# noamzilo/sed-crnn

Hardware: AMD Instinct MI355X
Metric: mel-frames/sec training throughput (seq=256, mel=40) (higher is better)
Workload: dtype f32; 1 GPU; BASELINE config 2: mono (B=128,256,40,1) per GPU, 3xConv3x3(128)+BN+ReLU+pool(1,2)+dropout0.5, BiGRU 2x128, Linear(256,1), BCEWithLogits, Adam lr 1e-3; full fit step (fwd+loss+bwd+allreduce+Adam); global_batch=128, seq_len=256, n_mels=40, parallelism=single

## Files before the change

sed_crnn_amd/csrc/conv1.hip:

```cpp
#include "common.h"

#define C1_TT 4
#define C1_MAXBLOCKS 2048

template <int CIN>
struct C1W { f32x4 w[9 * CIN]; f32x4 b; };

template <int CIN>
__device__ __forceinline__ void c1_load_w(C1W<CIN>& W, const float* __restrict__ wp, const float* __restrict__ bias,
                                          int Cout, int cg) {
#pragma unroll
    for (int tap = 0; tap < 9; ++tap)
#pragma unroll
        for (int ci = 0; ci < CIN; ++ci)
#pragma unroll
            for (int k = 0; k < 4; ++k) W.w[tap * CIN + ci][k] = wp[((size_t)tap * Cout + cg * 4 + k) * CIN + ci];
    W.b = bias ? *(const f32x4*)(bias + cg * 4) : (f32x4){0, 0, 0, 0};
}

template <int CIN>
__device__ __forceinline__ f32x4 c1_conv(const C1W<CIN>& W, const float* __restrict__ halo, int tl, int f, int F2) {
    f32x4 acc = W.b;
#pragma unroll
    for (int kh = 0; kh < 3; ++kh)
// ... 588 lines not shown
        const int k = areal[ta] ? fi : 0, tap = k / CIN, ci = k - tap * CIN, kh = tap / 3, kw = tap - kh * 3;
        aoff[ta] = areal[ta] ? ((kw + kk) * F2 + kh) * CIN + ci : hn + (fi == NK ? 0 : 1);
    }
    f32x16 acc[NFT][CT];
#pragma unroll
    for (int ta = 0; ta < NFT; ++ta)
#pragma unroll
        for (int ct = 0; ct < CT; ++ct)
#pragma unroll
            for (int j = 0; j < 16; ++j) acc[ta][ct][j] = 0.f;
    if (tid == 0) { halo[hn] = 1.f; halo[hn + 1] = 0.f; }
    for (int tile = blockIdx.x; tile < ntiles; tile += gridDim.x) {
        const int b = tile / tblocks, t0 = (tile - b * tblocks) * C1_RM_GT;
        __syncthreads();
        for (int j = tid; j < hn; j += 256) {
            int tt = j % (C1_RM_GT + 2), ff = (j / (C1_RM_GT + 2)) % F2, ci = j / ((C1_RM_GT + 2) * F2);
            const int t = t0 + tt - 1, f = ff - 1;
            float v = 0.f;
            if (t >= 0 && t < T && f >= 0 && f < F) v = x[(((size_t)b * CIN + ci) * F + f) * T + t];
            halo[(tt * F2 + ff) * CIN + ci] = v;
        }
        __syncthreads();
        const int tp = (t0 >> 1) + wave;
        if (tp < Tp) {
            const size_t prow = ((size_t)b * Tp + tp) * F;
            const float* dp = dout + prow * C + cg + i;
            const float* pp = pooled + prow * C + cg + i;
            const unsigned char* bp = bits + prow * (C >> 2) + ((cg + i) >> 2);
            const int rowbase = (2 * wave) * F2 * CIN;
            float dv[D][CT], qv[D][CT];
            unsigned bv8[D][CT];
            auto load = [&](int slot, int f) {
                const int fc = f < F ? f : F - 1;
#pragma unroll
                for (int ct = 0; ct < CT; ++ct) {
                    dv[slot][ct] = dp[(size_t)fc * C + ct * 32];
                    qv[slot][ct] = pp[(size_t)fc * C + ct * 32];
                    bv8[slot][ct] = bp[(size_t)fc * (C >> 2) + ct * 8];
                }
            };
#pragma unroll
            for (int sl = 0; sl < D; ++sl) load(sl, sl);
            for (int f0 = 0; f0 < F; f0 += D) {
#pragma unroll
                for (int sl = 0; sl < D; ++sl) {
                    const int f = f0 + sl;
                    const int base = rowbase + (f < F ? f : F - 1) * CIN;
                    float a[NFT];
#pragma unroll
                    for (int ta = 0; ta < NFT; ++ta) a[ta] = halo[areal[ta] ? base + aoff[ta] : aoff[ta]];
#pragma unroll
                    for (int ct = 0; ct < CT; ++ct) {
                        const float bv = (f < F && qv[sl][ct] > 0.f && (int)((bv8[sl][ct] >> (i & 3)) & 1u) == kk) ? dv[sl][ct] * inv_keep : 0.f;
#pragma unroll
                        for (int ta = 0; ta < NFT; ++ta)
                            acc[ta][ct] = __builtin_amdgcn_mfma_f32_32x32x2f32(a[ta], bv, acc[ta][ct], 0, 0, 0);
                    }
                    load(sl, f + D);
                }
            }
        }
    }
    float* red = smem;
#pragma unroll
    for (int ta = 0; ta < NFT; ++ta)
#pragma unroll
        for (int ct = 0; ct < CT; ++ct) {
            __syncthreads();
#pragma unroll
            for (int j = 0; j < 16; ++j) red[(wave * 32 + (j & 3) + 8 * (j >> 2) + 4 * kk) * 32 + i] = acc[ta][ct][j];
            __syncthreads();
            for (int e = tid; e < 1024; e += 256) {
                const int row = e >> 5, col = e & 31, fi = 32 * ta + row;
                if (fi <= NK) {
                    const float sum = (red[e] + red[1024 + e]) + (red[2048 + e] + red[3072 + e]);
                    partials[((size_t)blockIdx.x * C + cg + ct * 32 + col) * NV + (fi == NK ? 0 : 1 + fi)] = sum;
                }
            }
        }
}

__device__ __forceinline__ int c1_gidx(int k, int k2, int NK) { return NK + k * NK - (k * (k - 1)) / 2 + (k2 - k); }

__global__ __launch_bounds__(256) void conv1_wgrad_assemble_k(
    const float* __restrict__ part, int rows, int Cin, int C, const double* __restrict__ gram, const float* __restrict__ wp,
    const float* __restrict__ bias, const float* __restrict__ mean, const float* __restrict__ rstd, const float* __restrict__ scale,
    const float* __restrict__ sum_g, const float* __restrict__ sum_gx, double count, float* __restrict__ dw, float* __restrict__ db,
    const float* __restrict__ gamma, const float* __restrict__ beta, float* __restrict__ dgamma) {
    const int co = blockIdx.x, NK = 9 * Cin, NV = 1 + NK;
    __shared__ double sv[37];
    __shared__ double sw[4][37];
    const int lane = threadIdx.x & 63, wv = threadIdx.x >> 6;
    {
        double a[37];
#pragma unroll
        for (int v = 0; v < 37; ++v) a[v] = 0.0;
        for (int r = threadIdx.x; r < rows; r += 256) {
            const float* pr = part + ((size_t)r * C + co) * NV;
#pragma unroll
            for (int v = 0; v < 37; ++v)
                if (v < NV) a[v] += (double)pr[v];
        }
#pragma unroll
        for (int v = 0; v < 37; ++v) {
            if (v < NV) {
                const double t = wave_sum_d(a[v]);
                if (lane == 0) sw[wv][v] = t;
            }
        }
    }
    __syncthreads();
    if (threadIdx.x < NV) sv[threadIdx.x] = (sw[0][threadIdx.x] + sw[1][threadIdx.x]) + (sw[2][threadIdx.x] + sw[3][threadIdx.x]);
    __syncthreads();
    if (wv != 0) return;
    const double b = bias ? (double)bias[co] : 0.0, mu = mean[co], rs = rstd[co], sc = scale[co];
    double wr = 0.0, ws1 = 0.0;
    for (int k2 = 0; k2 < NK; ++k2) {
        const double w2 = (double)wp[((size_t)(k2 / Cin) * C + co) * Cin + (k2 % Cin)];
        ws1 += w2 * gram[k2];
        wr += w2 * sv[1 + k2];
    }
    const double sgx_sum = rs * (b * sv[0] + wr - mu * sv[0]);
    const bool own = sum_gx == nullptr;
    const double sg = (double)sum_g[co] / count, sgx = (own ? sgx_sum : (double)sum_gx[co]) / count;
    if (lane < NK) {
        const int k = lane;
        double wg = 0.0;
        for (int k2 = 0; k2 < NK; ++k2) {
            const double w2 = (double)wp[((size_t)(k2 / Cin) * C + co) * Cin + (k2 % Cin)];
            wg += w2 * gram[k <= k2 ? c1_gidx(k, k2, NK) : c1_gidx(k2, k, NK)];
        }
        const double s1 = gram[k];
        const double val = sc * (sv[1 + k] - sg * s1 - sgx * rs * (b * s1 + wg - mu * s1));
        const int tap = k / Cin, ci = k - tap * Cin;
        dw[((size_t)co * Cin + ci) * 9 + tap] = (float)val;
    }
    if (lane == 63) {
        const double sum_y = count * b + ws1;
        db[co] = (float)(sc * (sv[0] - count * sg - sgx * rs * (sum_y - count * mu)));
        if (dgamma && (own || (gamma && beta && gamma[co] == 0.f && beta[co] > 0.f))) dgamma[co] = (float)sgx_sum;
    }
}

static size_t c1_lds(int Cin, int F, int C, int mode) {
    size_t halo = (size_t)(C1_TT + 2) * (F + 2) * Cin * sizeof(float);
    size_t nv = mode == 3 ? 5 : 2;
    size_t red = (size_t)256 * 4 * nv * sizeof(float);
    return halo > red ? halo : red;
}

static int c1_shape_ok(int Cin, int F, int T, int C, int pool_f, int pool_t, int max_cin);
extern "C" int sed_conv1_fused_supported(int Cin, int F, int T, int C, int pool_f, int pool_t) {
    return c1_shape_ok(Cin, F, T, C, pool_f, pool_t, 2);
}
static int c1_shape_ok(int Cin, int F, int T, int C, int pool_f, int pool_t, int max_cin) {
    if (Cin < 1 || Cin > max_cin || C < 4 || F < 1 || T < 1 || C % 4 != 0 || C / 4 > 256 || (256 % (C / 4)) != 0) return 0;
    if (pool_t < 1 || pool_f < 1 || C1_TT % pool_t != 0 || T % C1_TT != 0 || F % pool_f != 0 || T % pool_t != 0) return 0;
    if (c1_lds(Cin, F, C, 3) > 150 * 1024) return 0;
    return 1;
}

extern "C" int sed_conv1_fused_rows(int B, int T) {
    long n = (long)B * ((T + C1_TT - 1) / C1_TT);
    return (int)(n < C1_MAXBLOCKS ? n : C1_MAXBLOCKS);
}

template <int MODE>
static int c1_launch(const float* x, const float* wp, const float* bias, const float* scale, const float* shift,
                     const float* mean, const float* rstd, const float* sum_g, const float* sum_gx, const float* dout,
                     float* out, float* partials, int B, int Cin, int F, int T, int C, int pf, int pt, float drop_p,
                     uint64_t seed, const uint64_t* seed_dev, hipStream_t s) {
    size_t lds = c1_lds(Cin, F, C, MODE);
    int grid = sed_conv1_fused_rows(B, T);
    const bool p12 = (pf == 1 && pt == 2);
#define C1_LAUNCH(CIN_, P12_)                                                                                          \
    do {                                                                                                               \
        if (lds > 48 * 1024)                                                                                           \
            (void)hipFuncSetAttribute((const void*)conv1_fused_k<CIN_, MODE, P12_>, hipFuncAttributeMaxDynamicSharedMemorySize, (int)lds); \
        conv1_fused_k<CIN_, MODE, P12_><<<grid, 256, lds, s>>>(x, wp, bias, scale, shift, mean, rstd, sum_g, sum_gx, dout, out, \
                                                              partials, B, F, T, C, pf, pt, drop_p, seed, seed_dev);  \
    } while (0)
    if (Cin == 1) { if (p12) C1_LAUNCH(1, true); else C1_LAUNCH(1, false); }
    else if (Cin == 2) { if (p12) C1_LAUNCH(2, true); else C1_LAUNCH(2, false); }
    else if ((MODE == 1 || MODE == 4) && p12) {
        if (Cin == 3) C1_LAUNCH(3, true);
        else C1_LAUNCH(4, true);
    } else {
        sed_set_error("conv1: %d input channels are supported by the forward pass with the (1,2) pool only", Cin);
        return SED_EUNSUPPORTED;
    }
#undef C1_LAUNCH
    return 0;
}
// ... 201 lines not shown
```

sed_crnn_amd/csrc/net.hip:

```cpp
#include <string.h>
#include "common.h"

namespace {

struct ConvL { int Cin, C, T, F, Tp, Fp, pf, pt, rows, bn_rows, nchw, fused; float drop;
               int red_rows;
               int rg_rows;
               int rgrad;
               int wino, wino_d;
               int ev;
               int bf; };

struct GruL { int in, H; };

struct Layout {
    int n_conv, n_gru, n_dense, M, Tp, Fp, feat;
    int proj_bf;
    ConvL cv[SED_MAX_CONV];
    GruL gr[SED_MAX_GRU];
    int dK[SED_MAX_DENSE], dN[SED_MAX_DENSE];
    size_t wp_f[SED_MAX_CONV], wp_d[SED_MAX_CONV], conv_out[SED_MAX_CONV], stat[SED_MAX_CONV];
    size_t mean[SED_MAX_CONV], rstd[SED_MAX_CONV], scale[SED_MAX_CONV], shift[SED_MAX_CONV];
    size_t pooled[SED_MAX_CONV], bn_sums[SED_MAX_CONV], c1_stat_ws, c1_bits, c1_mom;
    size_t bias_f[SED_MAX_CONV];
// ... 441 lines not shown
    for (int l = 0; l < L.n_conv; ++l) conv_bf16[l] = L.cv[l].bf;
    *proj_bf16 = L.proj_bf;
    return 0;
}

extern "C" int sed_net_routing(const sed_net_cfg* c, const sed_net_params* p, const float* x, const void* workspace, int block,
                               unsigned char* route, void* stream) {
    SED_REQUIRE(p && x && workspace && route, "net_routing: null pointer");
    Layout L;
    SED_TRY(build_layout(c, 1, &L));
    SED_REQUIRE(block >= 0 && block < L.n_conv, "net_routing: block %d out of range", block);
    const float* ws = (const float*)workspace;
    const ConvL& q = L.cv[block];
    if (q.fused) {
        SED_REQUIRE(p->conv_b[block], "net_routing: missing parameters of conv block %d", block);
        return sed_conv1_route(x, ws + L.wp_f[block], p->conv_b[block], ws + L.scale[block], ws + L.shift[block], route,
                               c->B, q.Cin, q.F, q.T, q.C, q.pf, q.pt, stream);
    }
    return sed_bn_relu_pool_route(ws + L.conv_out[block], ws + L.scale[block], ws + L.shift[block], route,
                                  c->B, q.T, q.F, q.C, q.pf, q.pt, stream);
}

static int bn_backward(const Layout& L, const sed_net_cfg* c, const sed_net_params* p, const sed_net_params* g,
                       const float* x, float* ws, uint64_t seed, const uint64_t* seed_dev, int l, int part, float count_scale, void* st) {
    const ConvL& q = L.cv[l];
    const int B = c->B, last = (l == L.n_conv - 1);
    const uint64_t sd = layer_seed(seed, l);
    SED_REQUIRE(g->conv_w[l] && g->conv_b[l] && g->bn_g[l] && g->bn_b[l], "net_backward: missing gradient buffers of conv block %d", l);
    float* sum_g = ws + L.sum_g;
    float* sum_gx = sum_g + q.C;
    if ((part & 1) && q.red_rows > 0 && !q.fused) {
        SED_TRY(sed_bn_bwd_finalize_small_gamma(ws + L.bn_part, q.red_rows, q.C, sum_g, sum_gx, g->bn_g[l], g->bn_b[l], ws + L.gradA,
                                                ws + L.pooled[l], ws + L.conv_out[l], p->bn_g[l], p->bn_b[l], ws + L.mean[l], ws + L.rstd[l],
                                                ws + L.scale[l], ws + L.shift[l], B, q.T, q.F, q.pf, q.pt, q.drop, st));
    } else if ((part & 1) && q.red_rows > 0) {
        SED_TRY(sed_bn_bwd_finalize(ws + L.bn_part, q.red_rows, q.C, sum_g, sum_gx, g->bn_g[l], g->bn_b[l], st));
    } else if (part & 1) {
        if (q.fused)
            SED_TRY(sed_conv1_bwd_reduce(x, ws + L.wp_f[l], p->conv_b[l], ws + L.gradA, ws + L.scale[l], ws + L.shift[l],
                                         ws + L.mean[l], ws + L.rstd[l], ws + L.bn_part, B, q.Cin, q.F, q.T, q.C, q.pf, q.pt,
                                         q.drop, sd, seed_dev, st));
        else if (sed_bn_bwd_reduce_pooled_supported(q.F, q.C, q.pf, q.pt, last))
            SED_TRY(sed_bn_bwd_reduce_pooled(ws + L.pooled[l], ws + L.gradA, p->bn_g[l], p->bn_b[l], ws + L.conv_out[l],
                                             ws + L.mean[l], ws + L.rstd[l], ws + L.scale[l], ws + L.shift[l], ws + L.bn_part, B, q.T, q.F, q.C, q.pf, q.pt, last, q.drop, st));
        else
            SED_TRY(sed_bn_relu_pool_drop_bwd_reduce(ws + L.conv_out[l], ws + L.gradA, ws + L.scale[l], ws + L.shift[l],
                                                     ws + L.mean[l], ws + L.rstd[l], ws + L.bn_part, B, q.T, q.F, q.C, q.pf,
                                                     q.pt, last, q.drop, sd, seed_dev, st));
        SED_TRY(sed_bn_bwd_finalize(ws + L.bn_part, q.bn_rows, q.C, sum_g, sum_gx, g->bn_g[l], g->bn_b[l], st));
    }
    if (part & 2) {
        if (count_scale != 1.f) SED_TRY(sed_scale(sum_g, 2 * q.C, 1.f / count_scale, st));
        if (q.fused && q.rgrad && q.rg_rows > 0) {
            SED_TRY(sed_conv1_bwd_wgrad_assemble(ws + L.c1_ws, q.rg_rows, (const double*)(ws + L.c1_mom), ws + L.wp_f[l], p->conv_b[l],
                                                 ws + L.mean[l], ws + L.rstd[l], ws + L.scale[l], sum_g, count_scale == 1.f ? nullptr : sum_gx, g->conv_w[l], g->conv_b[l],
                                                 B, q.Cin, q.F, q.T, q.C, p->bn_g[l], p->bn_b[l], g->bn_g[l], st));
        } else if (q.fused && q.rgrad) {
            SED_TRY(sed_conv1_bwd_wgrad(x, ws + L.gradA, ws + L.pooled[l], (const unsigned char*)(ws + L.c1_bits), (const double*)(ws + L.c1_mom),
                                        ws + L.wp_f[l], p->conv_b[l], ws + L.mean[l], ws + L.rstd[l], ws + L.scale[l], sum_g,
                                        (count_scale == 1.f && q.red_rows > 0) ? nullptr : sum_gx,
                                        g->conv_w[l], g->conv_b[l], ws + L.c1_ws, B, q.Cin, q.F, q.T, q.C, q.drop,
                                        q.red_rows > 0 ? p->bn_g[l] : nullptr, q.red_rows > 0 ? p->bn_b[l] : nullptr,
                                        q.red_rows > 0 ? g->bn_g[l] : nullptr, st));
        } else if (q.fused) {
            SED_TRY(sed_conv1_bwd_apply_wgrad(x, ws + L.wp_f[l], p->conv_b[l], ws + L.gradA, ws + L.scale[l], ws + L.shift[l],
                                              ws + L.mean[l], ws + L.rstd[l], sum_g, sum_gx, g->conv_w[l], g->conv_b[l],
                                              ws + L.c1_ws, B, q.Cin, q.F, q.T, q.C, q.pf, q.pt, q.drop, sd, seed_dev,
                                              q.red_rows > 0 ? p->bn_g[l] : nullptr, q.red_rows > 0 ? p->bn_b[l] : nullptr,
                                              q.red_rows > 0 ? g->bn_g[l] : nullptr, st));
        } else {
            SED_TRY(sed_bn_relu_pool_drop_bwd_apply(ws + L.conv_out[l], ws + L.gradA, ws + L.scale[l], ws + L.shift[l],
                                                    ws + L.mean[l], ws + L.rstd[l], sum_g, sum_gx, ws + L.dconv[l],
                                                    ws + L.dbias_part, B, q.T, q.F, q.C, q.pf, q.pt, last, q.drop, sd, seed_dev, st));
            SED_TRY(sed_reduce_rows(ws + L.dbias_part, q.bn_rows, q.C, q.C, g->conv_b[l], st));
        }
    }
    return 0;
}

static int dgrad(const Layout& L, const sed_net_cfg* c, const sed_net_params* p, const float* x, float* ws, int l, void* st) {
    const ConvL& q = L.cv[l];
    const ConvL& u = L.cv[l - 1];
    if (u.rg_rows > 0 && q.wino_d)
        return sed_conv3x3_wino_dgrad_bnred_rg(ws + L.dconv[l], ws + L.wp_d[l], ws + L.gradA, ws + L.bn_part, ws + L.pooled[l - 1],
                                               p->bn_g[l - 1], p->bn_b[l - 1], ws + L.mean[l - 1], ws + L.rstd[l - 1], u.drop,
                                               x, u.Cin, (const unsigned char*)(ws + L.c1_bits), ws + L.c1_ws, c->B, q.C, q.F, q.T, q.Cin, st);
    if (u.rg_rows > 0)
        return sed_conv3x3_dgrad_bnred_rg(ws + L.dconv[l], ws + L.wp_d[l], ws + L.gradA, ws + L.bn_part, ws + L.pooled[l - 1],
                                          p->bn_g[l - 1], p->bn_b[l - 1], ws + L.mean[l - 1], ws + L.rstd[l - 1], u.drop,
                                          x, u.Cin, (const unsigned char*)(ws + L.c1_bits), ws + L.c1_ws, c->B, q.C, q.F, q.T, q.Cin, st);
    if (q.wino_d)
        return sed_conv3x3_wino_dgrad_bnred(ws + L.dconv[l], ws + L.wp_d[l], ws + L.gradA, ws + L.bn_part, ws + L.pooled[l - 1],
                                            p->bn_g[l - 1], p->bn_b[l - 1], u.fused ? nullptr : ws + L.conv_out[l - 1],
                                            ws + L.mean[l - 1], ws + L.rstd[l - 1], u.drop, u.pf, u.pt, u.F, u.T, c->B, q.C, q.F, q.T, q.Cin, st);
    if (u.red_rows > 0)
        return sed_conv3x3_dgrad_bnred(ws + L.dconv[l], ws + L.wp_d[l], ws + L.gradA, ws + L.bn_part, ws + L.pooled[l - 1],
                                       p->bn_g[l - 1], p->bn_b[l - 1],
                                       u.fused ? nullptr : ws + L.conv_out[l - 1],
                                       ws + L.mean[l - 1], ws + L.rstd[l - 1],
                                       u.drop, u.pf, u.pt, u.F, u.T, c->B, q.C, q.F, q.T, q.Cin, st);
    return sed_conv3x3_fwd_ex(ws + L.dconv[l], 0, ws + L.wp_d[l], nullptr, ws + L.gradA, nullptr, c->B, q.C, q.F, q.T, q.Cin, c->conv_mode, st);
}

extern "C" int sed_net_backward(const sed_net_cfg* c, const sed_net_params* p, const sed_net_params* g,
                                const float* x, const float* dlogits, void* workspace, uint64_t seed,
                                const uint64_t* seed_dev, int stage_begin, int stage_end, void* stream, void* aux_stream) {
    SED_REQUIRE(p && g && x && dlogits && workspace, "net_backward: null pointer");
    constexpr int kMaxDev = 16;
    static thread_local hipEvent_t ev_all[kMaxDev][2][SED_MAX_CONV] = {};
    static thread_local hipEvent_t ev_gru_all[kMaxDev][SED_MAX_GRU + 5] = {};
    hipStream_t s_main = as_stream(stream), s_aux = as_stream(aux_stream);
    hipEvent_t* ev_dg = nullptr;
    hipEvent_t* ev_bn = nullptr;
    hipEvent_t* ev_gru = nullptr;
    if (s_aux && s_aux != s_main) {
        int dev = 0;
        if (hipGetDevice(&dev) != hipSuccess || dev < 0 || dev >= kMaxDev) {
            sed_set_error("net_backward: device index %d outside [0,%d)", dev, kMaxDev);
            return SED_EINVAL;
        }
        ev_dg = ev_all[dev][0];
        ev_bn = ev_all[dev][1];
        ev_gru = ev_gru_all[dev];
        for (int i = 0; i < SED_MAX_GRU + 5; ++i)
            if (!ev_gru[i] && hipEventCreateWithFlags(&ev_gru[i], hipEventDisableTiming) != hipSuccess) {
                sed_set_error("net_backward: hipEventCreate failed");
                return SED_EINVAL;
            }
        for (int l = 0; l < SED_MAX_CONV; ++l)
            if (!ev_dg[l]) {
                if (hipEventCreateWithFlags(&ev_dg[l], hipEventDisableTiming) != hipSuccess ||
                    hipEventCreateWithFlags(&ev_bn[l], hipEventDisableTiming) != hipSuccess) {
                    sed_set_error("net_backward: hipEventCreate failed");
                    return SED_EINVAL;
                }
            }
    } else {
        s_aux = nullptr;
    }
    Layout L;
    SED_TRY(build_layout(c, 1, &L));
    SED_REQUIRE(stage_begin >= 0 && stage_end <= L.n_conv + 1 && stage_begin < stage_end,
                "net_backward: bad stage range [%d,%d)", stage_begin, stage_end);
    float* ws = (float*)workspace;
    const int B = c->B, M = L.M;

    const int wg_clean = ((L.wgrad_zrow > 0 && s_aux) ? SED_WGRAD_ZERO_ROW_CLEAN : 0) | ((c->flags & SED_NET_DIRECT_CONV) ? SED_WGRAD_DIRECT : 0);
    if (s_aux && stage_begin == 0 && L.n_conv > 1) {
        hipError_t e = hipEventRecord(ev_gru[SED_MAX_GRU + 4], s_main);
        if (e == hipSuccess) e = hipStreamWaitEvent(s_aux, ev_gru[SED_MAX_GRU + 4], 0);
        if (e == hipSuccess) e = hipMemsetAsync(ws + L.wg_arrive, 0, (64 + L.wgrad_zrow) * sizeof(float), s_aux);
        if (e == hipSuccess && L.wgrad_zrow > 0) e = hipMemsetAsync(ws + L.wgrad_ws_aux, 0, L.wgrad_zrow * sizeof(float), s_aux);
        if (e == hipSuccess) e = hipEventRecord(ev_gru[SED_MAX_GRU + 3], s_aux);
        if (e != hipSuccess) {
            sed_set_error("net_backward: clearing the weight-gradient zero rows failed: %s", hipGetErrorString(e));
            return (int)e;
        }
    }

    if (stage_begin == 0) {
        const float* gru_last = ws + L.gout[L.n_gru - 1];
        for (int j = L.n_dense - 1; j >= 0; --j) {
            const int last = (j == L.n_dense - 1);
            const float* xin = (j == 0) ? gru_last : ws + L.act[j - 1];
            float* dy = last ? const_cast<float*>(dlogits) : ws + L.dact[j];
            float* dx = (j == 0) ? ws + L.dgout[L.n_gru - 1] : ws + L.dact[j - 1];
            SED_REQUIRE(g->dense_w[j] && g->dense_b[j], "net_backward: missing gradient buffers of dense layer %d", j);
// ... 194 lines not shown
```

sed_crnn_amd/csrc/wino.hip:

```cpp
#include "common.h"
#include "conv_shared.h"
#include <type_traits>

#define WN_CIN 128
#define WN_NHMAX 14

typedef __attribute__((address_space(1))) const void* sed_gptr_t;
typedef __attribute__((address_space(3))) void* sed_lptr_t;

struct WinoGeo {
    int Fw;
    int ncg, Tw, ntile, nblk, TR, F2, H2, HR, nb8, ncoh, NH;
    float invFw, invF2;
    size_t lds;
    unsigned long long* dbg;
};

__global__ void conv_pack_wino_k(const float* __restrict__ w, float* __restrict__ uf, float* __restrict__ ud, int Cout, int Cin,
                                 const float* __restrict__ bias, const float* __restrict__ gamma, const float* __restrict__ beta,
                                 const float* __restrict__ rm, const float* __restrict__ rv, float eps, float* __restrict__ bias_out) {
    const int i = blockIdx.x * blockDim.x + threadIdx.x;
    if (gamma && i < Cout) {
        const float sc = gamma[i] / sqrtf(rv[i] + eps);
        bias_out[i] = (bias ? bias[i] : 0.f) * sc + (beta[i] - rm[i] * sc);
// ... 75 lines not shown
    constexpr int CIN = WN_CIN, NCHUNK = CIN / 32, NSTEP = 4 * NCHUNK;
    constexpr int HBUF = NH * 1024;
    constexpr bool RG = RGC > 0;
    static_assert(!RG || BNR, "the tap sums belong to the BatchNorm-backward epilogue");
    static_assert(!EV || !BNR, "the pooling epilogue belongs to the inference forward");
    extern __shared__ __attribute__((aligned(16))) float smem[];
    const int tid = threadIdx.x, lane = tid & 63, wave = __builtin_amdgcn_readfirstlane(tid >> 6);
    const int r = lane & 31, h = lane >> 5;
    unsigned long long tk0 = 0, tk1 = 0, tk2 = 0;
    if (geo.dbg) tk0 = __builtin_amdgcn_s_memrealtime();

    int blka, coh, b;
    {
        const int bx = blockIdx.x, by = blockIdx.y, nba = geo.nblk * geo.ncg;
        if ((gridDim.y & 7) == 0) {
            const int id = by * (int)gridDim.x + bx, xcd = id & 7, j = id >> 3;
            coh = j % geo.ncoh;
            const int jj = j / geo.ncoh;
            b = xcd + 8 * (jj / nba);
            blka = jj % nba;
        } else {
            coh = bx % geo.ncoh; blka = bx / geo.ncoh; b = by;
        }
    }
    const int blk = blka / geo.ncg, cgp = blka - blk * geo.ncg;
    const int fg0 = 2 * cgp * geo.Fw;
    const int Fw = geo.Fw, F2 = geo.F2, H2 = geo.H2, ntile = geo.ntile;
    const int q0 = blk * 64, ty0 = q0 / Fw;
    const int co0 = coh * 64;

    const int ra = wave == 0 ? 0 : (wave == 2 ? 2 : 1);
    const int rb = wave == 0 ? 2 : (wave == 1 ? 2 : (wave == 2 ? 1 : 3));
    const float sg = wave == 1 ? 1.f : -1.f;

    const float* hp[NH];
    {
        const int Q = lane >> 3, pp = lane & 7;
        const float* zrow = uq + (size_t)16 * CIN * Cout;
#pragma unroll
        for (int u = 0; u < NH; ++u) {
            const int P = (u * 4 + wave) * 8 + pp;
            const int tt = sed_fdiv(P, geo.invF2), cx = P - tt * F2;
            const int ff = cx < H2 ? 2 * cx : 2 * (cx - H2) + 1;
            const int t = 2 * ty0 - 1 + tt, f = fg0 + ff - 1;
            const bool in = P < geo.HR && t >= 0 && t < T && f >= 0 && f < F;
            hp[u] = in ? x + ((((size_t)b * T + t) * F + f) * CIN + Q * 4) : zrow + Q * 4;
        }
    }
    auto issue = [&](int cc, float* buf) {
#pragma unroll
        for (int u = 0; u < NH; ++u)
            __builtin_amdgcn_global_load_lds((sed_gptr_t)(hp[u] + cc * 32), (sed_lptr_t)(buf + (u * 4 + wave) * 256), 16, 0, 0);
    };
    issue(0, smem);
    __builtin_amdgcn_sched_barrier(0);

    int aoff[2][2][4];
#pragma unroll
    for (int mt = 0; mt < 2; ++mt) {
        int q = q0 + mt * 32 + r;
        q = q < ntile ? q : ntile - 1;
        const int ty = sed_fdiv(q, geo.invFw), tf = q - ty * Fw;
#pragma unroll
        for (int s = 0; s < 2; ++s)
#pragma unroll
            for (int c = 0; c < 4; ++c) {
                const int P = (2 * (ty - ty0) + (s ? rb : ra)) * F2 + tf + (c & 1) * H2 + (c >> 1);
                aoff[mt][s][c] = (P >> 3) * 256 + h * 32 + (P & 7) * 4;
            }
    }


    unsigned* rowtab = (unsigned*)(smem + (2 * HBUF > 32768 + 512 ? 2 * HBUF : 32768 + 512));
    unsigned* xofftab = rowtab + 64;
    float* xs = (float*)(xofftab + 64);
    const int XT = 4 * geo.TR + 2;
    if (tid < 64) {
        const int q = q0 + tid;
        const int ty = sed_fdiv(q < ntile ? q : 0, geo.invFw), tf = q - ty * Fw;
        rowtab[tid] = q < ntile ? (unsigned)(((EV ? ty : 2 * ty) * F + fg0 + 2 * tf) * Cout) * 4u : 0xFFFFFFFFu;
        if (RG) xofftab[tid] = (unsigned)((fg0 + 2 * tf) * XT + 4 * (ty - ty0));
    }
    if (RG) {
        for (int i = tid; i < (F + 2) * XT; i += 256) {
            const int ff = i / XT, tt = i - ff * XT;
            const int f = ff - 1, t = 4 * ty0 - 1 + tt;
            const bool in = f >= 0 && f < F && t >= 0 && t < br.Ty;
#pragma unroll
            for (int ci = 0; ci < RGC; ++ci)
                xs[ci * (F + 2) * XT + i] = in ? br.x1[(((size_t)b * RGC + ci) * F + f) * br.Ty + t] : 0.f;
        }
    }

    f32x16 acc[4][2][2];
#pragma unroll
    for (int nu = 0; nu < 4; ++nu)
#pragma unroll
        for (int mt = 0; mt < 2; ++mt)
#pragma unroll
            for (int nt = 0; nt < 2; ++nt)
#pragma unroll
                for (int j = 0; j < 16; ++j) acc[nu][mt][nt][j] = 0.f;

    const f32x4* wl = (const f32x4*)uq + (size_t)(coh * 16 + wave * 4) * (NCHUNK * 4 * 2 * 64);
    f32x4 bq[4][2];
    const unsigned lane16 = (unsigned)lane * 16u;
    auto load_b = [&](int nu, int st) {
#pragma unroll
        for (int nt = 0; nt < 2; ++nt)
            bq[nu][nt] = *(const f32x4*)((const char*)(wl + ((nu * NSTEP + st) * 2 + nt) * 64) + lane16);
    };
    static_assert(NH <= 16, "the patch DMA of a slice rides in every fourth slot of its first step");
    f32x2 vp[2][2][4][2];
    f32x4 raw[2][2][4];
    f32x2 up[2][4][2];
    const f32x2 sg2 = {sg, sg};
    auto slot_read = [&](const float* buf, int g, int i) {
        const int mt = i >> 3, s2 = (i >> 2) & 1, c = i & 3;
        raw[mt][s2][c] = *(const f32x4*)(buf + aoff[mt][s2][c] + g * 64);
    };
    auto slot_xform = [&](int k, f32x2 (&v)[2][4][2]) {
        const int mt = k >> 4, q = k & 15, hf = q & 1;
        if (q < 8) {
            const int c = q >> 1;
            const f32x2 da = hf ? __builtin_shufflevector(raw[mt][0][c], raw[mt][0][c], 2, 3) : __builtin_shufflevector(raw[mt][0][c], raw[mt][0][c], 0, 1);
            const f32x2 db = hf ? __builtin_shufflevector(raw[mt][1][c], raw[mt][1][c], 2, 3) : __builtin_shufflevector(raw[mt][1][c], raw[mt][1][c], 0, 1);
            up[mt][c][hf] = wn_pk_fma(sg2, db, da);
        } else {
            const int nu = (q - 8) >> 1;
            if (nu == 0) v[mt][0][hf] = wn_pk_sub(up[mt][0][hf], up[mt][2][hf]);
            else if (nu == 1) v[mt][1][hf] = wn_pk_add(up[mt][1][hf], up[mt][2][hf]);
            else if (nu == 2) v[mt][2][hf] = wn_pk_sub(up[mt][2][hf], up[mt][1][hf]);
            else v[mt][3][hf] = wn_pk_sub(up[mt][1][hf], up[mt][3][hf]);
        }
    };
    auto issue_one = [&](int cc, float* buf, int u) {
        __builtin_amdgcn_global_load_lds((sed_gptr_t)(hp[u] + cc * 32), (sed_lptr_t)(buf + (u * 4 + wave) * 256), 16, 0, 0);
    };

#pragma unroll
    for (int nu = 0; nu < 4; ++nu) load_b(nu, 0);
    __syncthreads();
#pragma unroll
    for (int i = 0; i < 16; ++i) slot_read(smem, 0, i);
#pragma unroll
    for (int k = 0; k < 32; ++k) slot_xform(k, vp[0]);
    if (geo.dbg) tk1 = __builtin_amdgcn_s_memrealtime();
#pragma unroll
    for (int st = 0; st < NSTEP; ++st) {
        const int cc = st >> 2, g = st & 3, par = st & 1;
        const bool more = cc + 1 < NCHUNK, nxt = st + 1 < NSTEP;
        const float* nbuf = smem + (((st + 1) >> 2) & 1) * HBUF;
        __builtin_amdgcn_sched_barrier(0);
#pragma unroll
        for (int i = 0; i < 64; ++i) {
            const int nu = i >> 4, j = (i >> 2) & 3, mt = (i >> 1) & 1, nt = i & 1;
            acc[nu][mt][nt] = __builtin_amdgcn_mfma_f32_32x32x2f32(vp[par][mt][nu][j >> 1][j & 1], bq[nu][nt][j], acc[nu][mt][nt], 0, 0, 0);
            if (nxt && !(ABL & 4)) {
                if (i < 16) slot_read(nbuf, (st + 1) & 3, i);
                else if (i < 48 && !(ABL & 1)) slot_xform(i - 16, vp[par ^ 1]);
            }
            if (nxt && (i & 15) == 15 && !(ABL & 2)) load_b(nu, st + 1);
            if (g == 0 && more && !(ABL & 8) && (i & 3) == 1 && (i >> 2) < NH) issue_one(cc + 1, smem + ((cc + 1) & 1) * HBUF, i >> 2);
            __builtin_amdgcn_sched_barrier(0);
        }
        if (nxt && (ABL & 5)) {
#pragma unroll
            for (int a = 0; a < 2; ++a)
#pragma unroll
                for (int c = 0; c < 4; ++c) { vp[par ^ 1][a][c][0] = vp[par][a][c][0]; vp[par ^ 1][a][c][1] = vp[par][a][c][1]; }
        }
        if (g == 2 && more) __syncthreads();
    }
    __syncthreads();
    if (geo.dbg) tk2 = __builtin_amdgcn_s_memrealtime();

#pragma unroll
    for (int mt = 0; mt < 2; ++mt)
#pragma unroll
        for (int nt = 0; nt < 2; ++nt) {
            const f32x16 z0 = acc[0][mt][nt] + acc[1][mt][nt] + acc[2][mt][nt];
            const f32x16 z1 = acc[1][mt][nt] - acc[2][mt][nt] - acc[3][mt][nt];
            float* zb0 = smem + ((((wave * 2 + 0) * 2 + mt) * 2 + nt) << 10);
            float* zb1 = smem + ((((wave * 2 + 1) * 2 + mt) * 2 + nt) << 10);
#pragma unroll
            for (int j = 0; j < 16; ++j) {
                const int row = (j & 3) + 8 * (j >> 2) + 4 * h;
                zb0[row * 32 + r] = z0[j];
                zb1[row * 32 + r] = z1[j];
            }
        }
    __builtin_amdgcn_sched_barrier(0);
    const int mt = wave >> 1, nt = wave & 1;
    const int rq = lane >> 3, c4 = (lane & 7) * 4;
    const int cb = co0 + nt * 32 + c4;
    f32x4 bv = {0, 0, 0, 0};
    if (bias) bv = *(const f32x4*)(bias + cb);
    char* const yb = (char*)(y + (size_t)b * (EV ? T >> 1 : T) * F * Cout + cb);
    const char* const qb = BNR ? (const char*)(br.pooled + (size_t)b * T * F * Cout + cb) : nullptr;
    f32x4 q_kr = {0, 0, 0, 0}, q_nb = {0, 0, 0, 0}, a1 = {0, 0, 0, 0}, a2 = {0, 0, 0, 0};
    if (BNR) {
        const f32x4 q_beta = *(const f32x4*)(br.beta + cb);
        const f32x4 gm = *(const f32x4*)(br.gamma + cb);
#pragma unroll
        for (int e = 0; e < 4; ++e) {
            const bool zero = gm[e] == 0.f || (br.ybelow != nullptr && fabsf(gm[e]) * 64.f < fabsf(q_beta[e]));
            const float rg = zero ? 0.f : 1.0f / gm[e];
            q_kr[e] = br.keep * rg;
            q_nb[e] = -q_beta[e] * rg;
        }
    }
    const unsigned rstride = (unsigned)(F * Cout) * 4u, cstride = (unsigned)Cout * 4u;
    f32x4 R[RG ? 9 * RGC : 1];
#pragma unroll
    for (int k = 0; k < (RG ? 9 * RGC : 1); ++k) R[k] = (f32x4){0, 0, 0, 0};
    const unsigned char* const bitq = RG ? br.bits + (size_t)b * T * F * (Cout >> 2) + (cb >> 2) : nullptr;
    unsigned rov[4], xov[4];
#pragma unroll
    for (int k = 0; k < 4; ++k) {
        rov[k] = rowtab[mt * 32 + rq + 8 * k];
        xov[k] = RG ? xofftab[mt * 32 + rq + 8 * k] : 0u;
    }
    constexpr int PF = RGC == 2 ? 2 : 4;
    f32x4 pqv[PF][BNR ? 4 : 1];
    unsigned btv[PF][RG ? 4 : 1];
    auto prefetch = [&](int k, f32x4* pqd, unsigned* btd) {
        if (!BNR) return;
#pragma unroll
        for (int jj = 0; jj < 2; ++jj)
#pragma unroll
            for (int i = 0; i < 2; ++i) {
                const unsigned off = rov[k] + i * rstride + jj * cstride;
                pqd[jj * 2 + i] = (f32x4){0, 0, 0, 0};
                if (RG) btd[jj * 2 + i] = 0u;
                if (rov[k] != 0xFFFFFFFFu) {
                    pqd[jj * 2 + i] = *(const f32x4*)(qb + off);
                    if (RG) btd[jj * 2 + i] = bitq[off >> 4];
                }
            }
    };
    if (PF == 4) {
#pragma unroll
        for (int k = 0; k < 4; ++k) prefetch(k, pqv[k], btv[k]);
    } else prefetch(0, pqv[0], btv[0]);

    __syncthreads();
#pragma unroll
    for (int k = 0; k < 4; ++k) {
        const int m = rq + 8 * k;
        const unsigned ro = rov[k];
        if (PF == 2 && k + 1 < 4) prefetch(k + 1, pqv[(k + 1) & 1], btv[(k + 1) & 1]);
        if (ro == 0xFFFFFFFFu) continue;
        const unsigned xo = xov[k];
#pragma unroll
        for (int jj = 0; jj < 2; ++jj) {
            f32x4 z[4];
#pragma unroll
            for (int xi = 0; xi < 4; ++xi) z[xi] = *(const f32x4*)(smem + ((((xi * 2 + jj) * 2 + mt) * 2 + nt) << 10) + m * 32 + c4);
            const f32x4 o[2] = {z[0] + z[1] + z[2] + bv, z[1] - z[2] - z[3] + bv};
            if (EV) {
                f32x4 pl;
#pragma unroll
                for (int e = 0; e < 4; ++e) pl[e] = fmaxf(fmaxf(o[0][e], o[1][e]), 0.f);
                *(f32x4*)(yb + ro + jj * cstride) = pl;
                continue;
            }
#pragma unroll
            for (int i = 0; i < 2; ++i) {
                const unsigned off = ro + i * rstride + jj * cstride;
                const f32x4 v = o[i];
                *(f32x4*)(yb + off) = v;
                if (BNR) {
                    const f32x4 pq = pqv[k & (PF - 1)][jj * 2 + i];
                    f32x4 g0;
#pragma unroll
                    for (int e = 0; e < 4; ++e) g0[e] = pq[e] > 0.f ? v[e] : 0.f;
                    a1 += g0;
                    a2 += g0 * (pq * q_kr + q_nb);
                    if (RG) {
                        const unsigned bt = btv[k & (PF - 1)][jj * 2 + i];
                        f32x4 g1;
#pragma unroll
                        for (int e = 0; e < 4; ++e) g1[e] = ((bt >> e) & 1u) ? g0[e] : 0.f;
                        const f32x4 gA = g0 - g1;
#pragma unroll
                        for (int ci = 0; ci < RGC; ++ci) {
                            const float* xb = xs + ci * (F + 2) * XT + xo + jj * XT + 2 * i;
#pragma unroll
                            for (int kh = 0; kh < 3; ++kh) {
                                const f32x2 x01 = *(const f32x2*)(xb + kh * XT), x23 = *(const f32x2*)(xb + kh * XT + 2);
                                R[(kh * 3 + 0) * RGC + ci] += gA * x01[0] + g1 * x01[1];
                                R[(kh * 3 + 1) * RGC + ci] += gA * x01[1] + g1 * x23[0];
                                R[(kh * 3 + 2) * RGC + ci] += gA * x23[0] + g1 * x23[1];
                            }
                        }
                    }
                } else {
                    a1 += v;
                    a2 += v * v;
                }
            }
        }
    }
    if (stat && !EV) {
        float* red = smem + 32768;
        if (BNR) { a1 *= br.inv_keep; a2 *= br.inv_keep; }
#pragma unroll
        for (int e = 0; e < 4; ++e) {
#pragma unroll
            for (int o = 8; o < 64; o <<= 1) { a1[e] += __shfl_xor(a1[e], o, 64); a2[e] += __shfl_xor(a2[e], o, 64); }
        }
        if (lane < 8) {
            *(f32x4*)(red + (wave * 2 + 0) * 32 + c4) = a1;
            *(f32x4*)(red + (wave * 2 + 1) * 32 + c4) = a2;
        }
        float* red2 = xs + RGC * (F + 2) * XT;
        if (RG) {
#pragma unroll
            for (int k = 0; k < 9 * RGC; ++k) {
                R[k] *= br.inv_keep;
#pragma unroll
                for (int e = 0; e < 4; ++e) {
#pragma unroll
                    for (int o = 8; o < 64; o <<= 1) R[k][e] += __shfl_xor(R[k][e], o, 64);
                }
                if (lane < 8) *(f32x4*)(red2 + (wave * 9 * RGC + k) * 32 + c4) = R[k];
            }
        }
        __syncthreads();
        const size_t row = (size_t)b * geo.nblk * geo.ncg + blka;
        if (tid < 128) {
            const int which = tid >> 6, c = tid & 63, cn = c >> 5, cr = c & 31;
            const float a = red[((0 * 2 + cn) * 2 + which) * 32 + cr] + red[((1 * 2 + cn) * 2 + which) * 32 + cr];
            stat[row * 2 * Cout + which * Cout + co0 + c] = a;
        }
        if (RG && tid < 64) {
            const int cn = tid >> 5, cr = tid & 31;
            float* o = br.rgp + (row * Cout + co0 + tid) * (1 + 9 * RGC);
            o[0] = red[((0 * 2 + cn) * 2 + 0) * 32 + cr] + red[((1 * 2 + cn) * 2 + 0) * 32 + cr];
#pragma unroll
            for (int k = 0; k < 9 * RGC; ++k)
                o[1 + k] = red2[((0 * 2 + cn) * 9 * RGC + k) * 32 + cr] + red2[((1 * 2 + cn) * 9 * RGC + k) * 32 + cr];
        }
    }
    if (geo.dbg && tid == 0) {
        const unsigned long long tk3 = __builtin_amdgcn_s_memrealtime();
        atomicAdd(geo.dbg + 0, tk1 - tk0);
        atomicAdd(geo.dbg + 1, tk2 - tk1);
        atomicAdd(geo.dbg + 2, tk3 - tk2);
        atomicAdd(geo.dbg + 3, 1ull);
    }
}

template <typename K>
static int wino_set_lds(K kernel, size_t bytes) {
    hipError_t e = hipFuncSetAttribute((const void*)kernel, hipFuncAttributeMaxDynamicSharedMemorySize, (int)bytes);
    if (e != hipSuccess) { sed_set_error("hipFuncSetAttribute(%zu B LDS): %s", bytes, hipGetErrorString(e)); return (int)e; }
    return 0;
}

static unsigned long long* g_wino_dbg = nullptr;
#ifdef WN_ABLATION
static int g_wino_abl = 0;
extern "C" int sed_conv3x3_wino_ablate(int mask) { g_wino_abl = mask; return 0; }
#endif
extern "C" int sed_conv3x3_wino_phase_ticks(unsigned long long* buf) { g_wino_dbg = buf; return 0; }

int sed_internal_wino_launch(const float* x, const float* uq, const float* bias, float* y, float* stat, const ConvBnRed* br,
                             int rgc, int B, int Cin, int F, int T, int Cout, hipStream_t s) {
    WinoGeo g;
    SED_REQUIRE(wino_geo(B, Cin, F, T, Cout, &g), "conv3x3_wino: shape B=%d Cin=%d F=%d T=%d Cout=%d is not supported (sed_conv3x3_wino_rows)", B, Cin, F, T, Cout);
    SED_REQUIRE(rgc >= -1 && rgc <= 2 && (rgc <= 0 || (br && br->x1 && br->bits && br->rgp)) && (rgc >= 0 || (!br && !stat)), "conv3x3_wino: bad epilogue arguments");
    g.dbg = g_wino_dbg;
    if (rgc > 0) {
        g.lds += ((size_t)64 + (size_t)rgc * (F + 2) * (4 * g.TR + 2) + (size_t)4 * 9 * rgc * 32) * sizeof(float);
        SED_REQUIRE(g.lds <= 160 * 1024, "conv3x3_wino: the first block's input patch does not fit the LDS (F=%d)", F);
    }
    const dim3 grid(g.nblk * g.ncg * g.ncoh, B);
    const ConvBnRed none{};
#define WN_LAUNCH(NHv, BNRv, RGv, EVv)                                                                                          \
    do {                                                                                                                           \
        SED_TRY(wino_set_lds((conv3x3_wino_k<NHv, BNRv, RGv, EVv>), g.lds));                                                       \
        conv3x3_wino_k<NHv, BNRv, RGv, EVv><<<grid, 256, g.lds, s>>>(x, uq, bias, y, stat, B, F, T, Cout, g, br ? *br : none);     \
    } while (0)
#ifdef WN_ABLATION
    if (g_wino_abl && rgc == 0 && !br) {
        switch (g_wino_abl) {
            case 1: { SED_TRY(wino_set_lds((conv3x3_wino_k<WN_NHMAX, false, 0, false, 1>), g.lds)); conv3x3_wino_k<WN_NHMAX, false, 0, false, 1><<<grid, 256, g.lds, s>>>(x, uq, bias, y, stat, B, F, T, Cout, g, none); break; }
            case 2: { SED_TRY(wino_set_lds((conv3x3_wino_k<WN_NHMAX, false, 0, false, 2>), g.lds)); conv3x3_wino_k<WN_NHMAX, false, 0, false, 2><<<grid, 256, g.lds, s>>>(x, uq, bias, y, stat, B, F, T, Cout, g, none); break; }
            case 4: { SED_TRY(wino_set_lds((conv3x3_wino_k<WN_NHMAX, false, 0, false, 5>), g.lds)); conv3x3_wino_k<WN_NHMAX, false, 0, false, 5><<<grid, 256, g.lds, s>>>(x, uq, bias, y, stat, B, F, T, Cout, g, none); break; }
            case 8: { SED_TRY(wino_set_lds((conv3x3_wino_k<WN_NHMAX, false, 0, false, 8>), g.lds)); conv3x3_wino_k<WN_NHMAX, false, 0, false, 8><<<grid, 256, g.lds, s>>>(x, uq, bias, y, stat, B, F, T, Cout, g, none); break; }
            default: { SED_TRY(wino_set_lds((conv3x3_wino_k<WN_NHMAX, false, 0, false, 15>), g.lds)); conv3x3_wino_k<WN_NHMAX, false, 0, false, 15><<<grid, 256, g.lds, s>>>(x, uq, bias, y, stat, B, F, T, Cout, g, none); break; }
        }
        SED_LAUNCH_CHECK("conv3x3_wino (ablation)");
        return 0;
    }
#endif
    if (rgc == 1) WN_LAUNCH(WN_NHMAX, true, 1, false);
    else if (rgc == 2) WN_LAUNCH(WN_NHMAX, true, 2, false);
    else if (rgc == -1) WN_LAUNCH(WN_NHMAX, false, 0, true);
    else if (br) WN_LAUNCH(WN_NHMAX, true, 0, false);
    else WN_LAUNCH(WN_NHMAX, false, 0, false);
#undef WN_LAUNCH
    SED_LAUNCH_CHECK("conv3x3_wino");
    return 0;
}

extern "C" int sed_conv3x3_wino_rows(int B, int Cin, int F, int T, int Cout) { return sed_internal_wino_rows(B, Cin, F, T, Cout); }

extern "C" int sed_conv3x3_wino_fwd(const float* x, const float* uq, const float* bias, float* y, float* stat,
                                    int B, int Cin, int F, int T, int Cout, void* stream) {
    SED_REQUIRE(x && uq && y, "conv3x3_wino_fwd: null pointer");
    hipStream_t s = as_stream(stream);
    SedProfScope prof(SED_K_CONV_MFMA_FWD, s, 2.0 * 9.0 * Cin * Cout * (double)B * T * F);
    return sed_internal_wino_launch(x, uq, bias, y, stat, nullptr, 0, B, Cin, F, T, Cout, s);
}

extern "C" int sed_conv3x3_wino_dgrad_bnred(const float* dy, const float* ud, float* dx, float* partials, const float* pooled,
                                            const float* gamma, const float* beta, const float* conv_out_below, const float* mean,
                                            const float* rstd, float drop_p, int pool_f, int pool_t, int Fy, int Ty,
                                            int B, int C, int F, int T, int Cin, void* stream) {
    SED_REQUIRE(dy && ud && dx && partials && pooled && gamma && beta && mean && rstd, "conv3x3_wino_dgrad_bnred: null pointer");
    SED_REQUIRE(drop_p >= 0.f && drop_p < 1.f && pool_f >= 1 && pool_t >= 1, "conv3x3_wino_dgrad_bnred: bad drop_p / pool");
    SED_REQUIRE(Ty / pool_t == T && Fy / pool_f == F, "conv3x3_wino_dgrad_bnred: conv output %dx%d does not pool (%d,%d) to %dx%d", Ty, Fy, pool_f, pool_t, T, F);
    hipStream_t s = as_stream(stream);
    SedProfScope prof(SED_K_CONV_MFMA_DGRAD, s, 2.0 * 9.0 * C * Cin * (double)B * T * F);
    const ConvBnRed br{pooled, gamma, beta, conv_out_below, mean, rstd, 1.f - drop_p, 1.f / (1.f - drop_p), pool_f, pool_t, Fy, Ty,
                       nullptr, nullptr, nullptr, 0.f};
    return sed_internal_wino_launch(dy, ud, nullptr, dx, partials, &br, 0, B, C, F, T, Cin, s);
}

extern "C" int sed_conv3x3_wino_rg_rows(int B, int C, int F, int T, int Cin, int Cin1) {
    WinoGeo g;
    if (Cin1 < 1 || Cin1 > 2 || !wino_geo(B, C, F, T, Cin, &g)) return 0;
    const size_t lds = g.lds + ((size_t)64 + (size_t)Cin1 * (F + 2) * (4 * g.TR + 2) + (size_t)4 * 9 * Cin1 * 32) * sizeof(float);
    return lds <= 160 * 1024 ? B * g.nblk * g.ncg : 0;
}
extern "C" int sed_conv3x3_wino_dgrad_bnred_rg(const float* dy, const float* ud, float* dx, float* partials, const float* pooled,
                                               const float* gamma, const float* beta, const float* mean, const float* rstd, float drop_p,
                                               const float* x1, int Cin1, const unsigned char* argmax_bits, float* rg_partials,
                                               int B, int C, int F, int T, int Cin, void* stream) {
    SED_REQUIRE(dy && ud && dx && partials && pooled && gamma && beta && mean && rstd && x1 && argmax_bits && rg_partials, "conv3x3_wino_dgrad_bnred_rg: null pointer");
    SED_REQUIRE(drop_p >= 0.f && drop_p < 1.f && (Cin1 == 1 || Cin1 == 2), "conv3x3_wino_dgrad_bnred_rg: bad drop_p / input channels");
    hipStream_t s = as_stream(stream);
    SedProfScope prof(SED_K_CONV_MFMA_DGRAD, s, 2.0 * 9.0 * C * Cin * (double)B * T * F);
    const ConvBnRed br{pooled, gamma, beta, nullptr, mean, rstd, 1.f - drop_p, 1.f / (1.f - drop_p), 1, 2, F, 2 * T,
                       x1, argmax_bits, rg_partials, 0.f};
    return sed_internal_wino_launch(dy, ud, nullptr, dx, partials, &br, Cin1, B, C, F, T, Cin, s);
}

extern "C" int sed_conv3x3_wino_bn_relu_pool_eval(const float* x, const float* uf_folded, const float* bias_folded, float* pooled,
                                                  int B, int Cin, int F, int T, int Cout, void* stream) {
    SED_REQUIRE(x && uf_folded && bias_folded && pooled, "conv3x3_wino_bn_relu_pool_eval: null pointer");
    hipStream_t s = as_stream(stream);
    SedProfScope prof(SED_K_CONV_MFMA_FWD, s, 2.0 * 9.0 * Cin * Cout * (double)B * T * F);
    return sed_internal_wino_launch(x, uf_folded, bias_folded, pooled, nullptr, nullptr, -1, B, Cin, F, T, Cout, s);
}
```

Measured before the change: 5.702 million mel-frames/s.

## Overlap epilogue prefetch with last Winograd MFMA step and skip dead dx store

Peels the last MFMA step of the Winograd dgrad main loop and interleaves the epilogue's pooled/argmax-bit prefetches and gamma/beta loads with those MFMAs, so epilogue memory latency hides behind compute. When the layer below fuses its weight-gradient reduction, the dx output is passed as null and the kernel skips writing it. It also specialises the conv1 wgrad assemble row-sum loop per input-channel count with multi-row batching, and replaces an integer divide with a reciprocal multiply. These change scheduling and register pressure and rely on the dx buffer being truly unused downstream.

```diff
diff --git a/sed_crnn_amd/csrc/conv1.hip b/sed_crnn_amd/csrc/conv1.hip
--- a/sed_crnn_amd/csrc/conv1.hip
+++ b/sed_crnn_amd/csrc/conv1.hip
@@ -694,6 +694,38 @@
 
 __device__ __forceinline__ int c1_gidx(int k, int k2, int NK) { return NK + k * NK - (k * (k - 1)) / 2 + (k2 - k); }
 
+template <int NVT, int RB>
+__device__ __forceinline__ void c1_assemble_row_sums(const float* __restrict__ part, int rows, int C, int co, double (*sw)[37]) {
+    const int lane = threadIdx.x & 63, wv = threadIdx.x >> 6;
+    double a[NVT];
+#pragma unroll
+    for (int v = 0; v < NVT; ++v) a[v] = 0.0;
+    for (int r0 = threadIdx.x; r0 < rows; r0 += 256 * RB) {
+        float pv[RB][NVT];
+#pragma unroll
+        for (int u = 0; u < RB; ++u) {
+            const int r = r0 + 256 * u;
+            if (r < rows) {
+                const float* pr = part + ((size_t)r * C + co) * NVT;
+#pragma unroll
+                for (int v = 0; v < NVT; ++v) pv[u][v] = pr[v];
+            }
+        }
+#pragma unroll
+        for (int u = 0; u < RB; ++u) {
+            if (r0 + 256 * u < rows) {
+#pragma unroll
+                for (int v = 0; v < NVT; ++v) a[v] += (double)pv[u][v];
+            }
+        }
+    }
+#pragma unroll
+    for (int v = 0; v < NVT; ++v) {
+        const double t = wave_sum_d(a[v]);
+        if (lane == 0) sw[wv][v] = t;
+    }
+}
+
 __global__ __launch_bounds__(256) void conv1_wgrad_assemble_k(
     const float* __restrict__ part, int rows, int Cin, int C, const double* __restrict__ gram, const float* __restrict__ wp,
     const float* __restrict__ bias, const float* __restrict__ mean, const float* __restrict__ rstd, const float* __restrict__ scale,
@@ -703,24 +735,10 @@
     __shared__ double sv[37];
     __shared__ double sw[4][37];
     const int lane = threadIdx.x & 63, wv = threadIdx.x >> 6;
-    {
-        double a[37];
-#pragma unroll
-        for (int v = 0; v < 37; ++v) a[v] = 0.0;
-        for (int r = threadIdx.x; r < rows; r += 256) {
-            const float* pr = part + ((size_t)r * C + co) * NV;
-#pragma unroll
-            for (int v = 0; v < 37; ++v)
-                if (v < NV) a[v] += (double)pr[v];
-        }
-#pragma unroll
-        for (int v = 0; v < 37; ++v) {
-            if (v < NV) {
-                const double t = wave_sum_d(a[v]);
-                if (lane == 0) sw[wv][v] = t;
-            }
-        }
-    }
+    if (Cin == 1) c1_assemble_row_sums<10, 10>(part, rows, C, co, sw);
+    else if (Cin == 2) c1_assemble_row_sums<19, 5>(part, rows, C, co, sw);
+    else if (Cin == 3) c1_assemble_row_sums<28, 3>(part, rows, C, co, sw);
+    else c1_assemble_row_sums<37, 2>(part, rows, C, co, sw);
     __syncthreads();
     if (threadIdx.x < NV) sv[threadIdx.x] = (sw[0][threadIdx.x] + sw[1][threadIdx.x]) + (sw[2][threadIdx.x] + sw[3][threadIdx.x]);
     __syncthreads();
diff --git a/sed_crnn_amd/csrc/net.hip b/sed_crnn_amd/csrc/net.hip
--- a/sed_crnn_amd/csrc/net.hip
+++ b/sed_crnn_amd/csrc/net.hip
@@ -547,7 +547,7 @@
     const ConvL& q = L.cv[l];
     const ConvL& u = L.cv[l - 1];
     if (u.rg_rows > 0 && q.wino_d)
-        return sed_conv3x3_wino_dgrad_bnred_rg(ws + L.dconv[l], ws + L.wp_d[l], ws + L.gradA, ws + L.bn_part, ws + L.pooled[l - 1],
+        return sed_conv3x3_wino_dgrad_bnred_rg(ws + L.dconv[l], ws + L.wp_d[l], (u.fused && u.rgrad && u.rg_rows > 0) ? nullptr : ws + L.gradA, ws + L.bn_part, ws + L.pooled[l - 1],
                                                p->bn_g[l - 1], p->bn_b[l - 1], ws + L.mean[l - 1], ws + L.rstd[l - 1], u.drop,
                                                x, u.Cin, (const unsigned char*)(ws + L.c1_bits), ws + L.c1_ws, c->B, q.C, q.F, q.T, q.Cin, st);
     if (u.rg_rows > 0)
diff --git a/sed_crnn_amd/csrc/wino.hip b/sed_crnn_amd/csrc/wino.hip
--- a/sed_crnn_amd/csrc/wino.hip
+++ b/sed_crnn_amd/csrc/wino.hip
@@ -181,8 +181,9 @@
         if (RG) xofftab[tid] = (unsigned)((fg0 + 2 * tf) * XT + 4 * (ty - ty0));
     }
     if (RG) {
+        const float invXT = 1.0f / (float)XT;
         for (int i = tid; i < (F + 2) * XT; i += 256) {
-            const int ff = i / XT, tt = i - ff * XT;
+            const int ff = sed_fdiv(i, invXT), tt = i - ff * XT;
             const int f = ff - 1, t = 4 * ty0 - 1 + tt;
             const bool in = f >= 0 && f < F && t >= 0 && t < br.Ty;
 #pragma unroll
@@ -237,6 +238,33 @@
         __builtin_amdgcn_global_load_lds((sed_gptr_t)(hp[u] + cc * 32), (sed_lptr_t)(buf + (u * 4 + wave) * 256), 16, 0, 0);
     };
 
+    constexpr int PF = RGC == 2 ? 2 : 4;
+    int rq = 0, c4 = 0, cb = 0;
+    const char* qb = nullptr;
+    const unsigned char* bitq = nullptr;
+    unsigned rstride = 0, cstride = 0;
+    unsigned rov[4] = {0, 0, 0, 0};
+    f32x4 pqv[PF][BNR ? 4 : 1];
+    unsigned btv[PF][RG ? 4 : 1];
+    f32x4 q_beta = {0, 0, 0, 0}, gm = {0, 0, 0, 0};
+#define WN_EPI_LANE() do { rq = lane >> 3; c4 = (lane & 7) * 4; cb = co0 + nt * 32 + c4; } while (0)
+#define WN_EPI_STRIDES() do { rstride = (unsigned)(F * Cout) * 4u; cstride = (unsigned)Cout * 4u; } while (0)
+#define WN_EPI_ROWS() do { _Pragma("unroll") for (int k = 0; k < 4; ++k) rov[k] = rowtab[mt * 32 + rq + 8 * k]; } while (0)
+    auto epi_setup = [&]() {
+        const int mt = wave >> 1, nt = wave & 1;
+        WN_EPI_LANE();
+        qb = (const char*)(br.pooled + (size_t)b * T * F * Cout + cb);
+        bitq = RG ? br.bits + (size_t)b * T * F * (Cout >> 2) + (cb >> 2) : nullptr;
+        WN_EPI_STRIDES();
+        WN_EPI_ROWS();
+    };
+    auto prefetch_one = [&](int k, int n, f32x4* pqd, unsigned* btd) {
+        if (!BNR) return;
+        const unsigned off = rov[k] != 0xFFFFFFFFu ? rov[k] + (n & 1) * rstride + (n >> 1) * cstride : 0u;
+        pqd[n] = *(const f32x4*)(qb + off);
+        if (RG) btd[n] = bitq[off >> 4];
+    };
+
 #pragma unroll
     for (int nu = 0; nu < 4; ++nu) load_b(nu, 0);
     __syncthreads();
@@ -246,7 +274,7 @@
     for (int k = 0; k < 32; ++k) slot_xform(k, vp[0]);
     if (geo.dbg) tk1 = __builtin_amdgcn_s_memrealtime();
 #pragma unroll
-    for (int st = 0; st < NSTEP; ++st) {
+    for (int st = 0; st < (BNR ? NSTEP - 1 : NSTEP); ++st) {
         const int cc = st >> 2, g = st & 3, par = st & 1;
         const bool more = cc + 1 < NCHUNK, nxt = st + 1 < NSTEP;
         const float* nbuf = smem + (((st + 1) >> 2) & 1) * HBUF;
@@ -271,6 +299,20 @@
         }
         if (g == 2 && more) __syncthreads();
     }
+    if (BNR) {
+        constexpr int par = (NSTEP - 1) & 1;
+        epi_setup();
+        __builtin_amdgcn_sched_barrier(0);
+#pragma unroll
+        for (int i = 0; i < 64; ++i) {
+            const int nu = i >> 4, j = (i >> 2) & 3, mt = (i >> 1) & 1, nt = i & 1;
+            acc[nu][mt][nt] = __builtin_amdgcn_mfma_f32_32x32x2f32(vp[par][mt][nu][j >> 1][j & 1], bq[nu][nt][j], acc[nu][mt][nt], 0, 0, 0);
+            if (i < 4 * (PF == 4 ? 4 : 2)) prefetch_one(i >> 2, i & 3, pqv[i >> 2], btv[i >> 2]);
+            else if (i == 16) q_beta = *(const f32x4*)(br.beta + cb);
+            else if (i == 17) gm = *(const f32x4*)(br.gamma + cb);
+            __builtin_amdgcn_sched_barrier(0);
+        }
+    }
     __syncthreads();
     if (geo.dbg) tk2 = __builtin_amdgcn_s_memrealtime();
 
@@ -278,6 +320,10 @@
     for (int mt = 0; mt < 2; ++mt)
 #pragma unroll
         for (int nt = 0; nt < 2; ++nt) {
+            if (BNR) {
+#pragma unroll
+                for (int nu = 0; nu < 4; ++nu) asm volatile("" : "+a"(acc[nu][mt][nt]));
+            }
             const f32x16 z0 = acc[0][mt][nt] + acc[1][mt][nt] + acc[2][mt][nt];
             const f32x16 z1 = acc[1][mt][nt] - acc[2][mt][nt] - acc[3][mt][nt];
             float* zb0 = smem + ((((wave * 2 + 0) * 2 + mt) * 2 + nt) << 10);
@@ -288,19 +334,16 @@
                 zb0[row * 32 + r] = z0[j];
                 zb1[row * 32 + r] = z1[j];
             }
+            if (BNR) __builtin_amdgcn_sched_barrier(0);
         }
     __builtin_amdgcn_sched_barrier(0);
     const int mt = wave >> 1, nt = wave & 1;
-    const int rq = lane >> 3, c4 = (lane & 7) * 4;
-    const int cb = co0 + nt * 32 + c4;
+    if (!BNR) WN_EPI_LANE();
     f32x4 bv = {0, 0, 0, 0};
     if (bias) bv = *(const f32x4*)(bias + cb);
     char* const yb = (char*)(y + (size_t)b * (EV ? T >> 1 : T) * F * Cout + cb);
-    const char* const qb = BNR ? (const char*)(br.pooled + (size_t)b * T * F * Cout + cb) : nullptr;
     f32x4 q_kr = {0, 0, 0, 0}, q_nb = {0, 0, 0, 0}, a1 = {0, 0, 0, 0}, a2 = {0, 0, 0, 0};
     if (BNR) {
-        const f32x4 q_beta = *(const f32x4*)(br.beta + cb);
-        const f32x4 gm = *(const f32x4*)(br.gamma + cb);
 #pragma unroll
         for (int e = 0; e < 4; ++e) {
             const bool zero = gm[e] == 0.f || (br.ybelow != nullptr && fabsf(gm[e]) * 64.f < fabsf(q_beta[e]));
@@ -309,46 +352,28 @@
             q_nb[e] = -q_beta[e] * rg;
         }
     }
-    const unsigned rstride = (unsigned)(F * Cout) * 4u, cstride = (unsigned)Cout * 4u;
+    if (!BNR) WN_EPI_STRIDES();
     f32x4 R[RG ? 9 * RGC : 1];
 #pragma unroll
     for (int k = 0; k < (RG ? 9 * RGC : 1); ++k) R[k] = (f32x4){0, 0, 0, 0};
-    const unsigned char* const bitq = RG ? br.bits + (size_t)b * T * F * (Cout >> 2) + (cb >> 2) : nullptr;
-    unsigned rov[4], xov[4];
-#pragma unroll
-    for (int k = 0; k < 4; ++k) {
-        rov[k] = rowtab[mt * 32 + rq + 8 * k];
-        xov[k] = RG ? xofftab[mt * 32 + rq + 8 * k] : 0u;
-    }
-    constexpr int PF = RGC == 2 ? 2 : 4;
-    f32x4 pqv[PF][BNR ? 4 : 1];
-    unsigned btv[PF][RG ? 4 : 1];
+    if (!BNR) WN_EPI_ROWS();
+    unsigned xov[4];
+#pragma unroll
+    for (int k = 0; k < 4; ++k) xov[k] = RG ? xofftab[mt * 32 + rq + 8 * k] : 0u;
     auto prefetch = [&](int k, f32x4* pqd, unsigned* btd) {
-        if (!BNR) return;
-#pragma unroll
-        for (int jj = 0; jj < 2; ++jj)
-#pragma unroll
-            for (int i = 0; i < 2; ++i) {
-                const unsigned off = rov[k] + i * rstride + jj * cstride;
-                pqd[jj * 2 + i] = (f32x4){0, 0, 0, 0};
-                if (RG) btd[jj * 2 + i] = 0u;
-                if (rov[k] != 0xFFFFFFFFu) {
-                    pqd[jj * 2 + i] = *(const f32x4*)(qb + off);
-                    if (RG) btd[jj * 2 + i] = bitq[off >> 4];
-                }
-            }
-    };
-    if (PF == 4) {
-#pragma unroll
-        for (int k = 0; k < 4; ++k) prefetch(k, pqv[k], btv[k]);
-    } else prefetch(0, pqv[0], btv[0]);
+#pragma unroll
+        for (int n = 0; n < 4; ++n) prefetch_one(k, n, pqd, btd);
+    };
+    const bool wr_y = !RG || y != nullptr;
 
     __syncthreads();
+    unsigned long long tkx = 0;
+    if (BNR && geo.dbg) tkx = __builtin_amdgcn_s_memrealtime();
 #pragma unroll
     for (int k = 0; k < 4; ++k) {
         const int m = rq + 8 * k;
         const unsigned ro = rov[k];
-        if (PF == 2 && k + 1 < 4) prefetch(k + 1, pqv[(k + 1) & 1], btv[(k + 1) & 1]);
+        if (PF == 2 && k >= 1 && k + 1 < 4) prefetch(k + 1, pqv[(k + 1) & 1], btv[(k + 1) & 1]);
         if (ro == 0xFFFFFFFFu) continue;
         const unsigned xo = xov[k];
 #pragma unroll
@@ -368,7 +393,7 @@
             for (int i = 0; i < 2; ++i) {
                 const unsigned off = ro + i * rstride + jj * cstride;
                 const f32x4 v = o[i];
-                *(f32x4*)(yb + off) = v;
+                if (wr_y) *(f32x4*)(yb + off) = v;
                 if (BNR) {
                     const f32x4 pq = pqv[k & (PF - 1)][jj * 2 + i];
                     f32x4 g0;
@@ -448,8 +473,13 @@
         atomicAdd(geo.dbg + 1, tk2 - tk1);
         atomicAdd(geo.dbg + 2, tk3 - tk2);
         atomicAdd(geo.dbg + 3, 1ull);
-    }
-}
+        if (BNR) atomicAdd(geo.dbg + 4, tkx - tk2);
+    }
+}
+
+#undef WN_EPI_LANE
+#undef WN_EPI_STRIDES
+#undef WN_EPI_ROWS
 
 template <typename K>
 static int wino_set_lds(K kernel, size_t bytes) {
@@ -539,7 +569,7 @@
                                                const float* gamma, const float* beta, const float* mean, const float* rstd, float drop_p,
                                                const float* x1, int Cin1, const unsigned char* argmax_bits, float* rg_partials,
                                                int B, int C, int F, int T, int Cin, void* stream) {
-    SED_REQUIRE(dy && ud && dx && partials && pooled && gamma && beta && mean && rstd && x1 && argmax_bits && rg_partials, "conv3x3_wino_dgrad_bnred_rg: null pointer");
+    SED_REQUIRE(dy && ud && partials && pooled && gamma && beta && mean && rstd && x1 && argmax_bits && rg_partials, "conv3x3_wino_dgrad_bnred_rg: null pointer");
     SED_REQUIRE(drop_p >= 0.f && drop_p < 1.f && (Cin1 == 1 || Cin1 == 2), "conv3x3_wino_dgrad_bnred_rg: bad drop_p / input channels");
     hipStream_t s = as_stream(stream);
     SedProfScope prof(SED_K_CONV_MFMA_DGRAD, s, 2.0 * 9.0 * C * Cin * (double)B * T * F);
```

New measurement: 5.773 million mel-frames/s (median of 6 runs). 1.01x the previous value.
